# SYSTRAN/faster-whisper

Measured on AMD Instinct MI355X. Metric: audio-sec/sec (RTF) large-v3 fp16 beam=5 batch=16, higher is better.
Workload: dtype f16

## Files before the change

faster_whisper_amd/_lib.py:

```python
import ctypes as C
import os

import numpy as np

_HERE = os.path.dirname(os.path.abspath(__file__))
LIB_PATH = os.environ.get("FWAMD_LIB") or os.path.join(_HERE, "libfwamd.so")

FW_OK = 0
FW_EINVAL = -1
FW_ENODEV = -2
FW_ENOMEM = -3
FW_ERUNTIME = -4
FW_ENOSPC = -5

COMPUTE_FLOAT16 = 0
COMPUTE_INT8_FLOAT16 = 1
FW_DT_F32 = 0
FW_DT_F16 = 1
FW_MAX_ALIGN_HEADS = 64


class FwConfig(C.Structure):
    _fields_ = [
        ("n_mels", C.c_int32), ("n_audio_ctx", C.c_int32), ("d_model", C.c_int32), ("n_heads", C.c_int32),
        ("n_enc_layers", C.c_int32), ("n_dec_layers", C.c_int32), ("n_vocab", C.c_int32),
        ("n_text_ctx", C.c_int32), ("is_multilingual", C.c_int32),
        ("tok_eot", C.c_int32), ("tok_sot", C.c_int32), ("tok_lang_begin", C.c_int32), ("n_langs", C.c_int32),
        ("tok_translate", C.c_int32), ("tok_transcribe", C.c_int32), ("tok_sot_lm", C.c_int32),
        ("tok_sot_prev", C.c_int32), ("tok_no_speech", C.c_int32), ("tok_no_timestamps", C.c_int32),
        ("tok_timestamp_begin", C.c_int32),
        ("n_suppress_begin", C.c_int32), ("suppress_begin", C.c_int32 * 8),
        ("n_align_heads", C.c_int32), ("align_heads", C.c_int32 * (2 * FW_MAX_ALIGN_HEADS)),
    ]


class FwWeight(C.Structure):
    _fields_ = [("name", C.c_char_p), ("data", C.c_void_p), ("dtype", C.c_int32), ("ndim", C.c_int32),
                ("dims", C.c_int64 * 4)]


class FwGenOpts(C.Structure):
    _fields_ = [
        ("beam_size", C.c_int32), ("patience", C.c_float), ("num_hypotheses", C.c_int32),
        ("length_penalty", C.c_float), ("repetition_penalty", C.c_float), ("no_repeat_ngram_size", C.c_int32),
        ("max_length", C.c_int32), ("return_scores", C.c_int32), ("return_no_speech_prob", C.c_int32),
        ("max_initial_timestamp_index", C.c_int32), ("suppress_blank", C.c_int32),
        ("suppress_tokens", C.POINTER(C.c_int32)), ("n_suppress_tokens", C.c_int32),
        ("sampling_topk", C.c_int32), ("sampling_temperature", C.c_float), ("seed", C.c_uint64),
        ("min_new_tokens", C.c_int32),
    ]


class FwVadWeights(C.Structure):
    _fields_ = [
        ("stft_basis", C.c_void_p), ("conv_w", C.c_void_p * 4), ("conv_b", C.c_void_p * 4),
        ("lstm_w", C.c_void_p), ("lstm_r", C.c_void_p), ("lstm_b", C.c_void_p), ("dec_w", C.c_void_p),
        ("dec_b", C.c_float),
    ]


SYMBOLS = [
    "fw_last_error", "fw_abi_version", "fw_device_count",
    "fw_model_create", "fw_model_free", "fw_model_info", "fw_model_blob", "fw_model_create_from_blob_dev",
    "fw_model_set_decode_batch", "fw_model_decode_batch", "fw_model_join_decoder", "fw_model_decode_stats",
    "fw_model_set_merge_wait", "fw_model_set_decode_lanes", "fw_model_run_capacity", "fw_dec_big_min_rows", "fw_dec_big_min_rows_of", "fw_test_knob",
    "fw_test_idle_lead_chunks",
    "fw_pack_blob_size", "fw_pack_blob_copy", "fw_pack_blob_free",
    "fw_logmel", "fw_logmel_full",
    "fw_encode", "fw_encode_pcm", "fw_encode_pcm_dev", "fw_tensor_shape", "fw_tensor_to_host",
    "fw_tensor_from_host", "fw_tensor_free",
    "fw_generate", "fw_detect_language", "fw_align",
    "fw_prof_enable", "fw_prof_reset", "fw_prof_count", "fw_prof_name", "fw_prof_get", "fw_synchronize",
    "fw_dev_alloc", "fw_dev_free", "fw_dev_upload",
    "fw_test_gemm", "fw_test_layernorm", "fw_test_attention", "fw_test_dec_linear", "fw_test_dec_logits", "fw_test_logits_rules",
    "fw_test_dec_self_attn", "fw_test_dec_cross_attn", "fw_test_dec_cross_probs", "fw_test_dec_softmax_pick", "fw_bench_gemm", "fw_bench_dec_linear", "fw_bench_attention",
    "fw_bench_gemm_epi", "fw_bench_dec_linear_epi",
    "fw_vad_create", "fw_vad_forward", "fw_vad_free", "fw_vad_forward_dev", "fw_vad_forward_audio_dev",
    "fw_flac_info", "fw_flac_decode",
    "fw_resample_filter", "fw_resample_dev", "fw_bench_resample",
]

_lib = None


class FwError(RuntimeError):
    pass


def load():
    global _lib
    if _lib is not None:
        return _lib
    if not os.path.exists(LIB_PATH):
        raise FwError(
            f"{LIB_PATH} not found: build it with `python -c 'import __graft_entry__ as g; g.build()'` "
            "(hipcc --offload-arch=gfx950). faster_whisper_amd has no CPU fallback.")
    lib = C.CDLL(LIB_PATH)
    vp, i32, i64, f32p = C.c_void_p, C.c_int32, C.c_int64, C.POINTER(C.c_float)
    i32p, i64p = C.POINTER(C.c_int32), C.POINTER(C.c_int64)
    lib.fw_last_error.restype = C.c_char_p
    lib.fw_abi_version.restype = i32
    lib.fw_device_count.restype = i32
    lib.fw_model_create.argtypes = [C.POINTER(FwConfig), C.POINTER(FwWeight), i32, i32, i32, i32, i32, C.POINTER(vp)]
    lib.fw_model_free.argtypes = [vp]
    lib.fw_model_free.restype = None
    lib.fw_model_info.argtypes = [vp, C.POINTER(FwConfig), i32p, i32p, i32p, i32p]
    lib.fw_model_blob.argtypes = [vp, C.POINTER(vp), i64p]
    lib.fw_model_create_from_blob_dev.argtypes = [C.POINTER(FwConfig), vp, i64, i32, i32, i32, i32, C.POINTER(vp)]
    lib.fw_model_set_decode_batch.argtypes = [vp, i32]
    lib.fw_model_decode_batch.argtypes = [vp]
    lib.fw_model_decode_batch.restype = i32
    lib.fw_model_run_capacity.argtypes = [vp]
    lib.fw_model_run_capacity.restype = i32
    lib.fw_dec_big_min_rows.restype = i32
    if hasattr(lib, "fw_dec_big_min_rows_of"):
        lib.fw_dec_big_min_rows_of.restype = i32
        lib.fw_dec_big_min_rows_of.argtypes = [i32, i32]
    if hasattr(lib, "fw_flac_info"):
        lib.fw_flac_info.argtypes = [vp, i64, i32p, i32p, i32p, i64p]
        lib.fw_flac_decode.argtypes = [vp, i64, vp, i64, i64p, i32p]
    if hasattr(lib, "fw_test_knob"):
        lib.fw_test_knob.argtypes = [i32, i32]
    if hasattr(lib, "fw_test_idle_lead_chunks"):
        lib.fw_test_idle_lead_chunks.argtypes = [i64, i32, i32, i64, i32]
        lib.fw_test_idle_lead_chunks.restype = i64
    lib.fw_model_join_decoder.argtypes = [vp, vp]
    lib.fw_model_set_merge_wait.argtypes = [vp, i32, i32]
    lib.fw_model_set_decode_lanes.argtypes = [vp, i32]
    lib.fw_model_decode_stats.argtypes = [vp, i64p, i64p, i64p, i32p]
    lib.fw_pack_blob_size.argtypes = [C.POINTER(FwConfig), C.POINTER(FwWeight), i32, i32, i64p, C.POINTER(vp)]
    lib.fw_pack_blob_copy.argtypes = [vp, vp, i64]
    lib.fw_pack_blob_free.argtypes = [vp]
    lib.fw_pack_blob_free.restype = None
    lib.fw_logmel.argtypes = [vp, vp, i64p, i32, vp, i32p]
    lib.fw_logmel_full.argtypes = [vp, vp, i64, vp, i64]
    lib.fw_encode.argtypes = [vp, vp, i32, C.POINTER(vp)]
    lib.fw_encode_pcm.argtypes = [vp, vp, i64p, i32, C.POINTER(vp)]
    lib.fw_encode_pcm_dev.argtypes = [vp, vp, i64p, i32, C.POINTER(vp)]
    lib.fw_tensor_shape.argtypes = [vp, i32p, i32p, i32p]
    lib.fw_tensor_to_host.argtypes = [vp, vp, vp]
    lib.fw_tensor_from_host.argtypes = [vp, vp, i32, C.POINTER(vp)]
    lib.fw_tensor_free.argtypes = [vp]
    lib.fw_tensor_free.restype = None
    lib.fw_generate.argtypes = [vp, vp, i32p, i32p, i32, C.POINTER(FwGenOpts), i32p, i32p, f32p, f32p]
    lib.fw_detect_language.argtypes = [vp, vp, i32, i32p, f32p]
    lib.fw_align.argtypes = [vp, vp, i32p, i32, i32p, i32p, i32p, i32, i32, i32, i32p, i32p, f32p]
    lib.fw_prof_enable.argtypes = [vp, i32]
    lib.fw_prof_enable.restype = None
    lib.fw_prof_reset.argtypes = [vp]
    lib.fw_prof_reset.restype = None
    lib.fw_prof_count.restype = i32
    lib.fw_prof_name.argtypes = [i32]
    lib.fw_prof_name.restype = C.c_char_p
    lib.fw_prof_get.argtypes = [vp, i32, C.POINTER(C.c_double), i64p, C.POINTER(C.c_double), C.POINTER(C.c_double)]
    lib.fw_synchronize.argtypes = [vp]
    lib.fw_dev_alloc.argtypes = [vp, i64, C.POINTER(vp)]
    lib.fw_dev_free.argtypes = [vp, vp]
    lib.fw_dev_upload.argtypes = [vp, vp, vp, i64]
    lib.fw_test_gemm.argtypes = [vp, vp, vp, vp, vp, i32, i32, i32, i32, i32, vp]
    lib.fw_test_dec_linear.argtypes = [vp, vp, vp, vp, vp, vp, vp, i32, i32, i32, i32, i32, vp, vp]
    lib.fw_test_dec_logits.argtypes = [vp, vp, i32, vp]
    lib.fw_test_logits_rules.argtypes = [vp, vp, i32, vp, i32, vp, C.POINTER(FwGenOpts), i32, vp, vp]
    if hasattr(lib, "fw_test_dec_self_attn"):
        lib.fw_test_dec_self_attn.argtypes = [vp, vp, vp, vp, vp, i32, i32, i32, i32, i32, i32, i32, i32, i32, i32, i32, vp]
        lib.fw_test_dec_cross_attn.argtypes = [vp, vp, vp, vp, i32, i32, i32, i32, i32, i32, vp, vp, i32, C.c_float, vp]
        lib.fw_test_dec_cross_probs.argtypes = [vp, vp, vp, i32, i32, i32, vp, i32, i32, i32, i32, vp]
        lib.fw_test_dec_softmax_pick.argtypes = [vp, vp, i32, i32, i32, vp, i32, vp]
    lib.fw_bench_attention.argtypes = [vp, i32, i32, i32, i32, i32, f32p]
    lib.fw_bench_gemm.argtypes = [vp, i32, i32, i32, i32, i32, i32, i32, i32, f32p]
    lib.fw_bench_dec_linear.argtypes = [vp, i32, i32, i32, i32, i32, i32, f32p]
    if hasattr(lib, "fw_bench_gemm_epi"):
        lib.fw_bench_gemm_epi.argtypes = [vp, i32, i32, i32, i32, i32, i32, i32, i32, i32, i32, i32, f32p]
        lib.fw_bench_dec_linear_epi.argtypes = [vp, i32, i32, i32, i32, i32, i32, i32, i32, i32, f32p]
    lib.fw_test_layernorm.argtypes = [vp, vp, vp, vp, i32, i32, vp]
    lib.fw_test_attention.argtypes = [vp, vp, vp, vp, i32, i32, i32, vp]
    lib.fw_vad_create.argtypes = [C.POINTER(FwVadWeights), C.POINTER(vp)]
    lib.fw_vad_forward.argtypes = [vp, vp, i64, i32, vp, vp, vp]
    lib.fw_vad_free.argtypes = [vp]
    lib.fw_vad_forward_dev.argtypes = [vp, i32, vp, i64, vp, vp, vp]
    if hasattr(lib, "fw_vad_forward_audio_dev"):
        lib.fw_vad_forward_audio_dev.argtypes = [vp, i32, vp, i64, vp, vp, vp]
    lib.fw_vad_free.restype = None
    if hasattr(lib, "fw_resample_dev"):
        f64 = C.c_double
        lib.fw_resample_filter.argtypes = [i32, i32, i32, f64, vp, i64p, i32p, i32p]
        lib.fw_resample_dev.argtypes = [i32, vp, i64, i32, i32, i32, f64, i32, vp, i64]
        lib.fw_bench_resample.argtypes = [i32, vp, i64, i32, i32, i32, f64, i32, i32, f32p]
    _lib = lib
    return lib


def check(rc: int):
    if rc == FW_OK:
        return
    msg = load().fw_last_error().decode("utf-8", "replace")
    if rc in (FW_EINVAL, FW_ENOSPC):
        raise ValueError(msg)
    raise RuntimeError(f"libfwamd error {rc}: {msg}")


def ptr(a: np.ndarray):
    return a.ctypes.data_as(C.c_void_p)


def as_i32p(a: np.ndarray):
    return a.ctypes.data_as(C.POINTER(C.c_int32))


def as_i64p(a: np.ndarray):
    return a.ctypes.data_as(C.POINTER(C.c_int64))


def as_f32p(a: np.ndarray):
    return a.ctypes.data_as(C.POINTER(C.c_float))
```

faster_whisper_amd/csrc/dec_kernels.hip:

```cpp
#include "common.h"
#include "dec_kernels.h"
#include <stdlib.h>
#include <atomic>
#include <type_traits>

namespace fwd {
static std::atomic<int> g_self_attn_form{0};
static std::atomic<int> g_forms_epoch{0};
static std::atomic<int> g_cross_regs{0};
}

__device__ __forceinline__ size_t frag_off(int row, int k, int KS) {
  return ((size_t)((row >> 4) * KS + (k >> 5)) * 64 + ((k >> 3) & 3) * 16 + (row & 15)) * 8 + (k & 7);
}

__global__ void dec_embed_kernel(const int* __restrict__ tok, const half_t* __restrict__ emb,
                                 const half_t* __restrict__ pos_emb, half_t* __restrict__ x,
                                 half_t* __restrict__ xfrag, int d, const int* __restrict__ d_step, int pos_fixed,
                                 int P, int blk_n) {
  const int r = blockIdx.x;
  const int pos = blk_n > 0 ? pos_fixed + r % blk_n : (pos_fixed >= 0 ? pos_fixed : P - 1 + *d_step);
  const half2_t* e = reinterpret_cast<const half2_t*>(emb + (size_t)tok[r] * d);
  const half2_t* pe = reinterpret_cast<const half2_t*>(pos_emb + (size_t)pos * d);
  half2_t* xo = reinterpret_cast<half2_t*>(x + (size_t)r * d);
// ... 818 lines not shown
      src[j] = c * Kbeam + kvidx[pc];
      kv[j] = *reinterpret_cast<const half8_t*>(kbase + src[j] * slot_stride + (size_t)pc * 64);
    }
#pragma unroll
    for (int j = 0; j < 4; ++j) {
      const int p = p0 + 8 * j + pg;
      const float sc = dot8(kv[j]);
      if (p < pos) {
        if (cc == 0) { sp[p] = sc; ssrc[p] = src[j]; }
        mx = fmaxf(mx, sc);
      }
    }
  }
  mx = wave_max(mx);
  __builtin_amdgcn_wave_barrier();
  float sum = 0.f;
  for (int p = lane; p < pos; p += 64) {
    const float e = __expf(sp[p] - mx);
    sp[p] = e;
    sum += e;
  }
  const float e_new = __expf(s_new - mx);
  sum = wave_sum(sum) + e_new;
  __builtin_amdgcn_wave_barrier();
  float acc[8];
#pragma unroll
  for (int e = 0; e < 8; ++e) acc[e] = 0.f;
  const half_t* vb = vc + h * head_stride + cc * 8;
#pragma unroll 4
  for (int p = pg; p < pos; p += 8) {
    const half8_t vv = *reinterpret_cast<const half8_t*>(vb + ssrc[p] * slot_stride + (size_t)p * 64);
    const float w = sp[p];
#pragma unroll
    for (int e = 0; e < 8; ++e) acc[e] += w * (float)vv[e];
  }
#pragma unroll
  for (int e = 0; e < 8; ++e) {
    float a = acc[e];
    a += __shfl_xor(a, 8, 64);
    a += __shfl_xor(a, 16, 64);
    a += __shfl_xor(a, 32, 64);
    acc[e] = a;
  }
  if (pg == 0) {
    const float inv = 1.f / sum;
    half8_t o;
#pragma unroll
    for (int e = 0; e < 8; ++e) o[e] = (half_t)((acc[e] + e_new * (float)vn8[e]) * inv);
    half_t* dst = frag ? out + frag_off(r, h * 64 + cc * 8, d >> 5) : out + (size_t)r * d + h * 64 + cc * 8;
    *reinterpret_cast<half8_t*>(dst) = o;
  }
}

template <int U, bool PIPE, int MAXT, bool PB = false>
__global__ __launch_bounds__(MAXT) void dec_self_attn2_kernel(const half_t* __restrict__ qkv, int d, half_t* __restrict__ kc,
                                                             half_t* __restrict__ vc, int n_ctx, int cache_ctx,
                                                             int H, const uint8_t* __restrict__ kvidx2, int Kbeam, int kmul,
                                                             half_t* __restrict__ out, const int* __restrict__ d_step,
                                                             int pos_fixed, int P, int R_total, int frag) {
  extern __shared__ float sa_smem[];
  constexpr int NB = 4 * U;
  const int lane = threadIdx.x & 63;
  const int wave = __builtin_amdgcn_readfirstlane(threadIdx.x >> 6);
  float* sp = sa_smem + (size_t)wave * 2 * n_ctx;
  int* ssrc = reinterpret_cast<int*>(sp + n_ctx);
  const int h = blockIdx.x, c = blockIdx.y;
  const int r = c * kmul + wave, kb = PB ? 0 : wave;
  const int step = PB ? 0 : *d_step;
  const int pos = PB ? pos_fixed + wave : (pos_fixed >= 0 ? pos_fixed : P - 1 + step);
  const int slot = c * Kbeam + kb;
  const int cur = (pos_fixed >= 0) ? 0 : (step & 1);
  const uint8_t* kvidx = kvidx2 + ((size_t)cur * R_total + slot) * n_ctx;
  const half_t* qr = qkv + (size_t)r * 3 * d + h * 64;
  const size_t head_stride = (size_t)cache_ctx * 64;
  const size_t slot_stride = (size_t)H * head_stride;
  const int pg = lane >> 3, cc = lane & 7;
  for (int p4 = 4 * lane; p4 < pos; p4 += 256) {
    const unsigned w = PB ? 0u : *reinterpret_cast<const unsigned*>(kvidx + p4);
    intx4 s4;
    s4[0] = c * Kbeam + (int)(w & 0xffu); s4[1] = c * Kbeam + (int)((w >> 8) & 0xffu);
    s4[2] = c * Kbeam + (int)((w >> 16) & 0xffu); s4[3] = c * Kbeam + (int)(w >> 24);
    *reinterpret_cast<intx4*>(ssrc + p4) = s4;
  }
  const half8_t q8 = *reinterpret_cast<const half8_t*>(qr + cc * 8);
  const half8_t kn8 = *reinterpret_cast<const half8_t*>(qr + d + cc * 8);
  const half8_t vn8 = *reinterpret_cast<const half8_t*>(qr + 2 * d + cc * 8);
  float q[8];
#pragma unroll
  for (int e = 0; e < 8; ++e) q[e] = (float)q8[e] * 0.125f;
  if (pg == 0) {
    *reinterpret_cast<half8_t*>(kc + slot * slot_stride + h * head_stride + (size_t)pos * 64 + cc * 8) = kn8;
    *reinterpret_cast<half8_t*>(vc + slot * slot_stride + h * head_stride + (size_t)pos * 64 + cc * 8) = vn8;
  }
  auto dot8 = [&](const half8_t& k) {
    float sacc = 0.f;
#pragma unroll
    for (int e = 0; e < 8; ++e) sacc = __builtin_fmaf(q[e], (float)k[e], sacc);
    return sum8_dpp(sacc);
  };
  const float s_new = dot8(kn8);
  float mx = s_new;
  __builtin_amdgcn_wave_barrier();
  const char* kbase = reinterpret_cast<const char*>(kc + h * head_stride);
  const char* vbase = reinterpret_cast<const char*>(vc + h * head_stride);
  const unsigned slot_bytes = (unsigned)(slot_stride * sizeof(half_t));
  struct Batch { half8_t row[NB]; };
  auto fetch = [&](Batch& b, const char* base, int p0, const half_t* sib) {
#pragma unroll
    for (int j = 0; j < NB; ++j) {
      const int p = p0 + 8 * j + pg;
      const int pc = p < pos ? p : pos - 1;
      const unsigned off = (unsigned)ssrc[pc] * slot_bytes + (unsigned)(pc * 128 + cc * 16);
      if (PB && pc >= pos_fixed)
        b.row[j] = *reinterpret_cast<const half8_t*>(sib + (size_t)(pc - pos_fixed) * 3 * d + cc * 8);
      else
        b.row[j] = *reinterpret_cast<const half8_t*>(base + off);
    }
  };
  const half_t* ksib = qkv + (size_t)c * kmul * 3 * d + d + h * 64;
  const half_t* vsib = ksib + d;
  auto score = [&](const Batch& b, int p0) {
#pragma unroll
    for (int j = 0; j < NB; ++j) {
      const int p = p0 + 8 * j + pg;
      const float sc = dot8(b.row[j]);
      if (p < pos) {
        if (cc == 0) sp[p] = sc;
        mx = fmaxf(mx, sc);
      }
    }
  };
  Batch b0, b1;
  if (pos > 0) {
    fetch(b0, kbase, 0, ksib);
    for (int p0 = 0; p0 < pos; p0 += 16 * NB) {
      if (PIPE) {
        fetch(b1, kbase, p0 + 8 * NB, ksib);
        score(b0, p0);
        fetch(b0, kbase, p0 + 16 * NB, ksib);
        score(b1, p0 + 8 * NB);
      } else {
        score(b0, p0);
        if (p0 + 8 * NB < pos) {
          fetch(b0, kbase, p0 + 8 * NB, ksib);
          score(b0, p0 + 8 * NB);
          if (p0 + 16 * NB < pos) fetch(b0, kbase, p0 + 16 * NB, ksib);
        }
      }
    }
    fetch(b0, vbase, 0, vsib);
  }
  mx = wave_max_v(mx);
  __builtin_amdgcn_wave_barrier();
  float sum = 0.f;
  for (int p = lane; p < pos; p += 64) {
    const float e = __expf(sp[p] - mx);
    sp[p] = e;
    sum += e;
  }
  const float e_new = __expf(s_new - mx);
  sum = wave_sum_v(sum) + e_new;
  __builtin_amdgcn_wave_barrier();
  float acc[8];
#pragma unroll
  for (int e = 0; e < 8; ++e) acc[e] = 0.f;
  auto accum = [&](const Batch& b, int p0) {
#pragma unroll
    for (int j = 0; j < NB; ++j) {
      const int p = p0 + 8 * j + pg;
      if (p < pos) {
        const float w = sp[p];
#pragma unroll
        for (int e = 0; e < 8; ++e) acc[e] = __builtin_fmaf(w, (float)b.row[j][e], acc[e]);
      }
    }
  };
  for (int p0 = 0; p0 < pos; p0 += 16 * NB) {
    if (PIPE) {
      fetch(b1, vbase, p0 + 8 * NB, vsib);
      accum(b0, p0);
      fetch(b0, vbase, p0 + 16 * NB, vsib);
      accum(b1, p0 + 8 * NB);
    } else {
      accum(b0, p0);
      if (p0 + 8 * NB < pos) {
        fetch(b0, vbase, p0 + 8 * NB, vsib);
        accum(b0, p0 + 8 * NB);
        if (p0 + 16 * NB < pos) fetch(b0, vbase, p0 + 16 * NB, vsib);
      }
    }
  }
#pragma unroll
  for (int e = 0; e < 8; ++e) acc[e] = sum_x8_x16_x32_v(acc[e]);
  if (pg == 0) {
    const float inv = 1.f / sum;
    half8_t o;
#pragma unroll
    for (int e = 0; e < 8; ++e) o[e] = (half_t)((acc[e] + e_new * (float)vn8[e]) * inv);
    half_t* dst = frag ? out + frag_off(r, h * 64 + cc * 8, d >> 5) : out + (size_t)r * d + h * 64 + cc * 8;
    *reinterpret_cast<half8_t*>(dst) = o;
  }
}

template <int CA_WAVES, bool NTL, int MINW = 1>
__global__ __launch_bounds__(CA_WAVES * 64, MINW) void dec_cross_attn_kernel(const half_t* __restrict__ qx, int d,
                                                             const half_t* __restrict__ ck,
                                                             const half_t* __restrict__ cvt, int T, int kvp,
                                                             int kmul, half_t* __restrict__ out,
                                                             const int* __restrict__ done, int kv_div, int frag,
                                                             const int* __restrict__ slot_map) {
  __shared__ float sm[CA_WAVES][16], sl[CA_WAVES][16];
  __shared__ float so[CA_WAVES][16][65];
  const int h = blockIdx.x, c = blockIdx.y;
  if (done && done[c]) return;
  const int tid = threadIdx.x, lane = tid & 63, wave = tid >> 6;
  const int j = lane & 15, g = lane >> 4;
  const int ce = slot_map[c / kv_div];
  const half_t* kbase = ck + ((size_t)ce * (d >> 6) + h) * kvp * 64 + lane * 8;
  const half_t* vbase = cvt + ((size_t)ce * (d >> 6) + h) * kvp * 64 + lane * 8;
  half8_t qf[2];
  {
    if (j < kmul) {
      const half_t* qp = qx + (size_t)(c * kmul + j) * d + h * 64 + g * 8;
#pragma unroll
      for (int s = 0; s < 2; ++s) {
        half8_t v = *reinterpret_cast<const half8_t*>(qp + s * 32);
#pragma unroll
        for (int e = 0; e < 8; ++e) v[e] = v[e] * (half_t)0.125f;
        qf[s] = v;
      }
    } else {
      qf[0] = half8_t{0, 0, 0, 0, 0, 0, 0, 0};
      qf[1] = qf[0];
    }
  }
  floatx4 o[4];
#pragma unroll
  for (int dt = 0; dt < 4; ++dt) o[dt] = floatx4{0, 0, 0, 0};
  float m_run = -1.0e30f, l_run = 0.f;
  const float LOG2E = 1.4426950408889634f;
  const int ngroups = (T + 31) >> 5;
  auto load_kv = [&](int gi, half8_t (&kf)[4], half8_t (&vf)[4]) {
    const half_t* kp = kbase + (size_t)gi * 2048;
    const half_t* vp = vbase + (size_t)gi * 2048;
#pragma unroll
    for (int q = 0; q < 4; ++q)
      kf[q] = NTL ? __builtin_nontemporal_load(reinterpret_cast<const half8_t*>(kp + q * 512))
                  : *reinterpret_cast<const half8_t*>(kp + q * 512);
#pragma unroll
    for (int dt = 0; dt < 4; ++dt)
      vf[dt] = NTL ? __builtin_nontemporal_load(reinterpret_cast<const half8_t*>(vp + dt * 512))
// ... 670 lines not shown
    if (K >= 2560)
      dec_gemm_frag_i8_kernel<8, 4, 4, 3><<<g4, 512, 0, st>>>(xq, x_scale, Wq, w_scale, bias, res, ldr, out, ldo, R, N, K, act);
    else
      dec_gemm_frag_i8_kernel<4, 4, 4, 5><<<g4, 256, 0, st>>>(xq, x_scale, Wq, w_scale, bias, res, ldr, out, ldo, R, N, K, act);
    return 0;
  }
  const dim3 grid(N / 32, ((R + 15) / 16 + 1) / 2);
  if (K >= 2560)
    dec_gemm_frag_i8_kernel<8, 2, 2><<<grid, 512, 0, st>>>(xq, x_scale, Wq, w_scale, bias, res, ldr, out, ldo, R, N, K, act);
  else
    dec_gemm_frag_i8_kernel<4, 2, 2><<<grid, 256, 0, st>>>(xq, x_scale, Wq, w_scale, bias, res, ldr, out, ldo, R, N, K, act);
  return 0;
}

template <bool I8, bool LNF, int RT>
static void wave_go(hipStream_t st, const void* xf, const float* x_scale, const void* Wf, const float* w_scale,
                    const float* s1, const float* cf, float* out, int ldo, int R, int N, int K) {
  constexpr int NT = 2, WM = 1, WN = 4;
  const int n_rt = (R + 15) / 16, n_ct = (N + 15) / 16;
  const int n_cg = ((n_ct + NT * WN - 1) / (NT * WN) + 7) & ~7;
  const int n_rg = (n_rt + RT * WM - 1) / (RT * WM);
  dec_gemm_wave_kernel<I8, LNF, true, RT, NT, WM, WN><<<n_cg * n_rg, WM * WN * 64, 0, st>>>(
      xf, x_scale, Wf, w_scale, nullptr, s1, cf, out, ldo, R, N, K, n_rg);
}

int launch_dec_logits(hipStream_t st, bool i8, const void* xf, const float* x_scale, const void* Wf,
                      const float* w_scale, const float* s1, const float* cf, float* out, int ldo, int R, int N, int K) {
  if (K % (i8 ? 64 : 32) != 0 || R < 1) return -1;
  if (i8 ? (!x_scale || !w_scale) : ((s1 == nullptr) != (cf == nullptr))) return -1;
  const int n_rt = (R + 15) / 16;
#define WG(RT)                                                                                   \
  do {                                                                                           \
    if (i8) wave_go<true, false, RT>(st, xf, x_scale, Wf, w_scale, s1, cf, out, ldo, R, N, K);   \
    else if (s1) wave_go<false, true, RT>(st, xf, x_scale, Wf, w_scale, s1, cf, out, ldo, R, N, K); \
    else wave_go<false, false, RT>(st, xf, x_scale, Wf, w_scale, s1, cf, out, ldo, R, N, K);     \
  } while (0)
  if (n_rt == 1) WG(1);
  else if (n_rt == 2) WG(2);
  else if (n_rt == 3) WG(3);
  else if (n_rt == 4) WG(4);
  else WG(5);
#undef WG
  return 0;
}

bool self_attn_block_ok(int n_ctx, int cache_ctx, int d, int R_total) {
  return (n_ctx & 3) == 0 && (size_t)R_total * cache_ctx * d * sizeof(half_t) < ((size_t)1 << 32);
}

void launch_self_attn(hipStream_t st, const half_t* qkv, int d, half_t* kc, half_t* vc, int n_ctx, int cache_ctx, int H,
                      const uint8_t* kvidx2, int Kbeam, int kmul, half_t* out, int rows, const int* d_step,
                      int pos_fixed, int P, int R_total, int frag, int blk_n) {
  if (blk_n > 0) {
    dec_self_attn2_kernel<1, true, 1024, true><<<dim3(H, rows / blk_n), blk_n * 64, (size_t)blk_n * 2 * n_ctx * sizeof(float), st>>>(
        qkv, d, kc, vc, n_ctx, cache_ctx, H, kvidx2, Kbeam, blk_n, out, d_step, pos_fixed, P, R_total, frag);
    return;
  }
  const dim3 grid(H, rows / kmul);
  const size_t lds = (size_t)kmul * 2 * n_ctx * sizeof(float);
  int form = g_self_attn_form.load(std::memory_order_relaxed);
  if ((n_ctx & 3) != 0 || (size_t)R_total * cache_ctx * d * sizeof(half_t) >= ((size_t)1 << 32)) form = 1;
  if (form == 0) form = (kmul <= 8 && (int)(grid.x * grid.y) <= 768) ? 2 : 3;
  if (form == 2 && kmul > 8) form = 3;
#define SA_ARGS qkv, d, kc, vc, n_ctx, cache_ctx, H, kvidx2, Kbeam, kmul, out, d_step, pos_fixed, P, R_total, frag
  if (form == 1) dec_self_attn_kernel<<<grid, kmul * 64, lds, st>>>(SA_ARGS);
  else if (form == 2) dec_self_attn2_kernel<4, false, 512><<<grid, kmul * 64, lds, st>>>(SA_ARGS);
  else dec_self_attn2_kernel<1, true, 1024><<<grid, kmul * 64, lds, st>>>(SA_ARGS);
#undef SA_ARGS
}
void set_self_attn_form(int form) { g_self_attn_form.store(form); g_forms_epoch.fetch_add(1); }
int kernel_forms_epoch() { return g_forms_epoch.load(); }
void bump_kernel_forms_epoch() { g_forms_epoch.fetch_add(1); }

void launch_cross_attn(hipStream_t st, const half_t* qx, int d, const half_t* ck, const half_t* cvt, int T, int kvp,
                       int kmul, half_t* out, int B, int H, const int* done, int kv_div, int frag, const int* slot_map) {
  const int cap = g_cross_regs.load(std::memory_order_relaxed);
  if (cap == 1)
    dec_cross_attn_kernel<8, true, 5><<<dim3(H, B), 512, 0, st>>>(qx, d, ck, cvt, T, kvp, kmul, out, done, kv_div, frag, slot_map);
  else if (cap == 2)
    dec_cross_attn_kernel<8, true, 6><<<dim3(H, B), 512, 0, st>>>(qx, d, ck, cvt, T, kvp, kmul, out, done, kv_div, frag, slot_map);
  else
    dec_cross_attn_kernel<8, true><<<dim3(H, B), 512, 0, st>>>(qx, d, ck, cvt, T, kvp, kmul, out, done, kv_div, frag, slot_map);
}
void set_cross_attn_regs(int cap) { g_cross_regs.store(cap); g_forms_epoch.fetch_add(1); }

void launch_nospeech(hipStream_t st, const float* logits, int V, int row_mul, int no_speech_id, float* out, int B) {
  dec_nospeech_kernel<<<B, 1024, 0, st>>>(logits, V, row_mul, no_speech_id, out);
}

void launch_logits_process(hipStream_t st, const GenDev& gp, float* logits, const unsigned long long* sup_bits,
                           const int* hist2, const float* cum2, const int* d_step, const int* done, float* cand_val,
                           int* cand_tok) {
  const bool wide = gp.ts_begin >= 48 * LP_THREADS;
#define LP_GO(SMP, TXI) \
  dec_logits_process_kernel<SMP, TXI><<<gp.R, LP_THREADS, 0, st>>>(gp, logits, sup_bits, hist2, cum2, d_step, done, cand_val, cand_tok)
  if (gp.sample) { if (wide) LP_GO(true, 48); else LP_GO(true, 0); }
  else { if (wide) LP_GO(false, 48); else LP_GO(false, 0); }
#undef LP_GO
}

void launch_beam_update(hipStream_t st, const GenDev& gp, const float* cand_val, const int* cand_tok, int* hist2,
                        float* cum2, uint8_t* kvidx2, int* cur_tok, const int* d_step, int* done, int* n_done,
                        int* n_fin, int* fin_tok, int* fin_len, float* fin_score, float* fin_cum) {
  dec_beam_update_kernel<<<gp.B, 64, 0, st>>>(gp, cand_val, cand_tok, hist2, cum2, kvidx2, cur_tok, d_step, done,
                                              n_done, n_fin, fin_tok, fin_len, fin_score, fin_cum);
}

void launch_step_advance(hipStream_t st, int* d_step) { dec_step_advance_kernel<<<1, 1, 0, st>>>(d_step); }

void launch_token_prob(hipStream_t st, const float* logits, int V, const int* target, float* out, int out_stride,
                       int out_off, int rows, int row_mul) {
  dec_token_prob_kernel<<<rows, 1024, 0, st>>>(logits, V, target, out, out_stride, out_off, row_mul);
// ... 11 lines not shown
```

faster_whisper_amd/csrc/engine.hip:

```cpp
#include "engine.h"

#include <math.h>
#include <stdarg.h>
#include <stdio.h>
#include <stdlib.h>
#include <string.h>

#include <algorithm>

#include "dec_kernels.h"
#include "kernels.h"

namespace fw {

static thread_local char g_err[1024] = "";
void set_error(const char* fmt, ...) {
  va_list ap;
  va_start(ap, fmt);
  vsnprintf(g_err, sizeof(g_err), fmt, ap);
  va_end(ap);
}

int dev_alloc(void** p, size_t bytes) {
  if (bytes == 0) bytes = 256;
// ... 2163 lines not shown
  int rc;
  auto cleanup = [&]() { for (half_t* p : {dqk, dvt, dout}) if (p) (void)hipFree(p); };
  if ((rc = dev_alloc_t(&dqk, nqk)) || (rc = dev_alloc_t(&dvt, nvt)) || (rc = dev_alloc_t(&dout, no))) { cleanup(); return rc; }
  {
    std::vector<uint16_t> h(std::max(nqk, nvt));
    uint32_t sd = 777u;
    for (auto& v : h) { sd = sd * 1664525u + 1013904223u; v = f32_to_f16_bits(((int)(sd >> 16) % 2001 - 1000) * 2e-3f); }
    FW_HIP(hipMemcpy(dqk, h.data(), nqk * 2, hipMemcpyHostToDevice));
    FW_HIP(hipMemcpy(dvt, h.data(), nvt * 2, hipMemcpyHostToDevice));
  }
  hipEvent_t e0, e1;
  FW_HIP(hipEventCreate(&e0));
  FW_HIP(hipEventCreate(&e1));
  auto go = [&]() {
    fwk::launch_attn_enc(m->stream, dqk, dqk + d, 2 * d, (int64_t)T * 2 * d, dvt, tp, (int64_t)d * tp, dout, d, (int64_t)T * d, B,
                         H, T, variant);
  };
  go();
  FW_HIP(hipEventRecord(e0, m->stream));
  for (int i = 0; i < iters; ++i) go();
  FW_HIP(hipEventRecord(e1, m->stream));
  hipError_t he = hipEventSynchronize(e1);
  float ms = 0.f;
  if (he == hipSuccess) he = hipEventElapsedTime(&ms, e0, e1);
  (void)hipEventDestroy(e0);
  (void)hipEventDestroy(e1);
  cleanup();
  if (he != hipSuccess) { set_error("attention bench failed: %s", hipGetErrorString(he)); return FW_ERUNTIME; }
  *ms_out = ms / (float)iters;
  return FW_OK;
}

extern "C++" {
namespace {
struct DevBufs {
  std::vector<void*> p;
  template <typename T>
  int alloc(T** dst, size_t n) {
    int rc = dev_alloc_t(dst, n);
    if (!rc) p.push_back(*dst);
    return rc;
  }
  ~DevBufs() { for (void* q : p) (void)hipFree(q); }
};
int upload_f16_to(const float* src, size_t n, half_t* dst) {
  std::vector<uint16_t> tmp(n);
  for (size_t i = 0; i < n; ++i) tmp[i] = f32_to_f16_bits(src[i]);
  FW_HIP(hipMemcpy(dst, tmp.data(), n * 2, hipMemcpyHostToDevice));
  return FW_OK;
}
}
}

int32_t fw_test_dec_self_attn(fw_model* fm, const float* qkv, float* kcache, float* vcache, const uint8_t* kvidx,
                              int32_t n_chunks, int32_t kmul, int32_t Kbeam, int32_t H, int32_t n_ctx, int32_t cache_ctx,
                              int32_t pos_fixed, int32_t P, int32_t step, int32_t blk_n, int32_t frag, float* out) {
  FW_CHECK_ARG(fm && qkv && kcache && vcache && kvidx && out, "null argument");
  FW_CHECK_ARG(n_chunks >= 1 && H >= 1 && kmul >= 1 && kmul <= 16 && Kbeam >= 1 && Kbeam <= 255, "bad geometry");
  FW_CHECK_ARG(n_ctx >= 1 && n_ctx <= 448 && cache_ctx >= 1 && cache_ctx <= n_ctx, "need 1 <= cache_ctx <= n_ctx <= 448");
  FW_CHECK_ARG(blk_n >= 0 && (blk_n == 0 ? kmul <= Kbeam : (kmul == blk_n && pos_fixed >= 0)),
               "blk_n = 0: kmul <= Kbeam; blk_n > 0: kmul == blk_n and pos_fixed >= 0");
  const int pos0 = pos_fixed >= 0 ? pos_fixed : P - 1 + step;
  const int pos_last = pos0 + (blk_n > 0 ? blk_n - 1 : 0);
  FW_CHECK_ARG(pos0 >= 0 && pos_last < cache_ctx, "positions %d..%d outside the cache (%d)", pos0, pos_last, cache_ctx);
  const int d = H * 64, R = n_chunks * kmul, R16 = (R + 15) / 16 * 16, R_total = n_chunks * Kbeam;
  FW_CHECK_ARG(blk_n == 0 || fwd::self_attn_block_ok(n_ctx, cache_ctx, d, R_total), "position blocks need n_ctx %% 4 == 0");
  const size_t n_tab = (size_t)2 * R_total * n_ctx, n_cache = (size_t)R_total * H * cache_ctx * 64;
  for (size_t i = 0; i < n_tab; ++i)
    FW_CHECK_ARG(kvidx[i] < Kbeam, "kvidx[%zu] = %d is not a beam of %d", i, (int)kvidx[i], Kbeam);
  Model* m = &fm->impl;
  std::lock_guard<std::mutex> lk(m->mu);
  FW_HIP(hipSetDevice(m->device));
  DevBufs db;
  half_t *d_qkv, *d_kc, *d_vc, *d_out;
  uint8_t* d_idx;
  int* d_step;
  int rc;
  if ((rc = db.alloc(&d_qkv, (size_t)R * 3 * d)) || (rc = db.alloc(&d_kc, n_cache)) || (rc = db.alloc(&d_vc, n_cache)) ||
      (rc = db.alloc(&d_out, (size_t)R16 * d)) || (rc = db.alloc(&d_idx, n_tab)) || (rc = db.alloc(&d_step, 1)))
    return rc;
  if ((rc = upload_f16_to(qkv, (size_t)R * 3 * d, d_qkv)) || (rc = upload_f16_to(kcache, n_cache, d_kc)) ||
      (rc = upload_f16_to(vcache, n_cache, d_vc)))
    return rc;
  FW_HIP(hipMemcpy(d_idx, kvidx, n_tab, hipMemcpyHostToDevice));
  FW_HIP(hipMemcpy(d_step, &step, sizeof(int), hipMemcpyHostToDevice));
  FW_HIP(hipMemset(d_out, 0, (size_t)R16 * d * 2));
  fwd::launch_self_attn(m->stream, d_qkv, d, d_kc, d_vc, n_ctx, cache_ctx, H, d_idx, Kbeam, kmul, d_out, R, d_step,
                        pos_fixed, P, R_total, frag ? 1 : 0, blk_n);
  FW_HIP(hipGetLastError());
  if ((rc = download_f16(m, d_kc, n_cache, kcache)) || (rc = download_f16(m, d_vc, n_cache, vcache))) return rc;
  if (!frag) return download_f16(m, d_out, (size_t)R * d, out);
  std::vector<float> of((size_t)R16 * d);
  if ((rc = download_f16(m, d_out, of.size(), of.data()))) return rc;
  for (int r = 0; r < R; ++r)
    for (int n = 0; n < d; ++n) out[(size_t)r * d + n] = of[frag_pos(r, n, d, 32)];
  return FW_OK;
}

int32_t fw_test_dec_cross_attn(fw_model* fm, const float* q, const float* k, const float* v, int32_t n_enc, int32_t T,
                               int32_t H, int32_t B, int32_t kmul, int32_t kv_div, const int32_t* slot_map,
                               const int32_t* done, int32_t frag, float k_pad, float* out) {
  FW_CHECK_ARG(fm && q && k && v && slot_map && out, "null argument");
  FW_CHECK_ARG(n_enc >= 1 && T >= 1 && H >= 1 && B >= 1 && kmul >= 1 && kmul <= 16 && kv_div >= 1, "bad geometry");
  const int n_map = (B + kv_div - 1) / kv_div;
  for (int i = 0; i < n_map; ++i)
    FW_CHECK_ARG(slot_map[i] >= 0 && slot_map[i] < n_enc, "slot_map[%d] = %d outside [0, %d)", i, slot_map[i], n_enc);
// ... 99 lines not shown
```

Measured before the change: 3193.

## Precompute byte offsets in LDS table and trim decoder self-attention inner loop

```diff
diff --git a/faster_whisper_amd/_lib.py b/faster_whisper_amd/_lib.py
--- a/faster_whisper_amd/_lib.py
+++ b/faster_whisper_amd/_lib.py
@@ -74,7 +74,7 @@
     "fw_dev_alloc", "fw_dev_free", "fw_dev_upload",
     "fw_test_gemm", "fw_test_layernorm", "fw_test_attention", "fw_test_dec_linear", "fw_test_dec_logits", "fw_test_logits_rules",
     "fw_test_dec_self_attn", "fw_test_dec_cross_attn", "fw_test_dec_cross_probs", "fw_test_dec_softmax_pick", "fw_bench_gemm", "fw_bench_dec_linear", "fw_bench_attention",
-    "fw_bench_gemm_epi", "fw_bench_dec_linear_epi",
+    "fw_bench_gemm_epi", "fw_bench_dec_linear_epi", "fw_bench_dec_self_attn",
     "fw_vad_create", "fw_vad_forward", "fw_vad_free", "fw_vad_forward_dev", "fw_vad_forward_audio_dev",
     "fw_flac_info", "fw_flac_decode",
     "fw_resample_filter", "fw_resample_dev", "fw_bench_resample",
@@ -172,6 +172,8 @@
     if hasattr(lib, "fw_bench_gemm_epi"):
         lib.fw_bench_gemm_epi.argtypes = [vp, i32, i32, i32, i32, i32, i32, i32, i32, i32, i32, i32, f32p]
         lib.fw_bench_dec_linear_epi.argtypes = [vp, i32, i32, i32, i32, i32, i32, i32, i32, i32, f32p]
+    if hasattr(lib, "fw_bench_dec_self_attn"):
+        lib.fw_bench_dec_self_attn.argtypes = [vp, i32, i32, i32, i32, i32, i32, i32, f32p]
     lib.fw_test_layernorm.argtypes = [vp, vp, vp, vp, i32, i32, vp]
     lib.fw_test_attention.argtypes = [vp, vp, vp, vp, i32, i32, i32, vp]
     lib.fw_vad_create.argtypes = [C.POINTER(FwVadWeights), C.POINTER(vp)]
diff --git a/faster_whisper_amd/csrc/dec_kernels.hip b/faster_whisper_amd/csrc/dec_kernels.hip
--- a/faster_whisper_amd/csrc/dec_kernels.hip
+++ b/faster_whisper_amd/csrc/dec_kernels.hip
@@ -894,8 +894,10 @@
   }
 }
 
+static __host__ __device__ __forceinline__ int sa2_table_len(int n_ctx) { return ((n_ctx + 127) & ~127) + 32; }
+static __host__ __device__ __forceinline__ int sa2_lds_words(int n_ctx) { return ((n_ctx + 7) & ~7) + sa2_table_len(n_ctx); }
 template <int U, bool PIPE, int MAXT, bool PB = false>
-__global__ __launch_bounds__(MAXT) void dec_self_attn2_kernel(const half_t* __restrict__ qkv, int d, half_t* __restrict__ kc,
+__global__ __launch_bounds__(MAXT, (U == 1 && !PB) ? 8 : 1) void dec_self_attn2_kernel(const half_t* __restrict__ qkv, int d, half_t* __restrict__ kc,
                                                              half_t* __restrict__ vc, int n_ctx, int cache_ctx,
                                                              int H, const uint8_t* __restrict__ kvidx2, int Kbeam, int kmul,
                                                              half_t* __restrict__ out, const int* __restrict__ d_step,
@@ -904,8 +906,8 @@
   constexpr int NB = 4 * U;
   const int lane = threadIdx.x & 63;
   const int wave = __builtin_amdgcn_readfirstlane(threadIdx.x >> 6);
-  float* sp = sa_smem + (size_t)wave * 2 * n_ctx;
-  int* ssrc = reinterpret_cast<int*>(sp + n_ctx);
+  float* sp = sa_smem + (size_t)wave * sa2_lds_words(n_ctx);
+  int* ssrc = reinterpret_cast<int*>(sp + ((n_ctx + 7) & ~7));
   const int h = blockIdx.x, c = blockIdx.y;
   const int r = c * kmul + wave, kb = PB ? 0 : wave;
   const int step = PB ? 0 : *d_step;
@@ -916,13 +918,27 @@
   const half_t* qr = qkv + (size_t)r * 3 * d + h * 64;
   const size_t head_stride = (size_t)cache_ctx * 64;
   const size_t slot_stride = (size_t)H * head_stride;
+  const unsigned slot_bytes = (unsigned)(slot_stride * sizeof(half_t));
   const int pg = lane >> 3, cc = lane & 7;
-  for (int p4 = 4 * lane; p4 < pos; p4 += 256) {
-    const unsigned w = PB ? 0u : *reinterpret_cast<const unsigned*>(kvidx + p4);
-    intx4 s4;
-    s4[0] = c * Kbeam + (int)(w & 0xffu); s4[1] = c * Kbeam + (int)((w >> 8) & 0xffu);
-    s4[2] = c * Kbeam + (int)((w >> 16) & 0xffu); s4[3] = c * Kbeam + (int)(w >> 24);
-    *reinterpret_cast<intx4*>(ssrc + p4) = s4;
+  if constexpr (PB) {
+    for (int p4 = 4 * lane; p4 < pos; p4 += 256) {
+      intx4 s4;
+#pragma unroll
+      for (int i = 0; i < 4; ++i) s4[i] = (int)((unsigned)(c * Kbeam) * slot_bytes + (unsigned)(p4 + i) * 128u);
+      *reinterpret_cast<intx4*>(ssrc + p4) = s4;
+    }
+  } else if (pos > 0) {
+    const int ext = PIPE ? ((pos + 16 * NB - 1) & ~(16 * NB - 1)) + 8 * NB : (pos + 8 * NB - 1) & ~(8 * NB - 1);
+    const unsigned last = (unsigned)(c * Kbeam + kvidx[pos - 1]) * slot_bytes + (unsigned)(pos - 1) * 128u;
+    for (int p4 = 4 * lane; p4 < ext; p4 += 256) {
+      const unsigned w = p4 < pos ? *reinterpret_cast<const unsigned*>(kvidx + p4) : 0u;
+      intx4 s4;
+#pragma unroll
+      for (int i = 0; i < 4; ++i)
+        s4[i] = p4 + i < pos ? (int)((unsigned)(c * Kbeam + (int)((w >> (8 * i)) & 0xffu)) * slot_bytes + (unsigned)(p4 + i) * 128u)
+                             : (int)last;
+      *reinterpret_cast<intx4*>(ssrc + p4) = s4;
+    }
   }
   const half8_t q8 = *reinterpret_cast<const half8_t*>(qr + cc * 8);
   const half8_t kn8 = *reinterpret_cast<const half8_t*>(qr + d + cc * 8);
@@ -943,33 +959,47 @@
   const float s_new = dot8(kn8);
   float mx = s_new;
   __builtin_amdgcn_wave_barrier();
-  const char* kbase = reinterpret_cast<const char*>(kc + h * head_stride);
-  const char* vbase = reinterpret_cast<const char*>(vc + h * head_stride);
-  const unsigned slot_bytes = (unsigned)(slot_stride * sizeof(half_t));
+  const unsigned head_bytes = (unsigned)h * ((unsigned)cache_ctx * 128u);
+  const char* kbase = reinterpret_cast<const char*>(kc) + head_bytes;
+  const char* vbase = reinterpret_cast<const char*>(vc) + head_bytes;
   struct Batch { half8_t row[NB]; };
   auto fetch = [&](Batch& b, const char* base, int p0, const half_t* sib) {
 #pragma unroll
     for (int j = 0; j < NB; ++j) {
       const int p = p0 + 8 * j + pg;
-      const int pc = p < pos ? p : pos - 1;
-      const unsigned off = (unsigned)ssrc[pc] * slot_bytes + (unsigned)(pc * 128 + cc * 16);
-      if (PB && pc >= pos_fixed)
-        b.row[j] = *reinterpret_cast<const half8_t*>(sib + (size_t)(pc - pos_fixed) * 3 * d + cc * 8);
-      else
-        b.row[j] = *reinterpret_cast<const half8_t*>(base + off);
+      if constexpr (PB) {
+        const int pc = p < pos ? p : pos - 1;
+        if (pc >= pos_fixed)
+          b.row[j] = *reinterpret_cast<const half8_t*>(sib + (size_t)(pc - pos_fixed) * 3 * d + cc * 8);
+        else
+          b.row[j] = *reinterpret_cast<const half8_t*>(base + ((unsigned)ssrc[pc] + (unsigned)(cc * 16)));
+      } else {
+        b.row[j] = *reinterpret_cast<const half8_t*>(base + ((unsigned)ssrc[p] + (unsigned)(cc * 16)));
+      }
     }
   };
   const half_t* ksib = qkv + (size_t)c * kmul * 3 * d + d + h * 64;
   const half_t* vsib = ksib + d;
-  auto score = [&](const Batch& b, int p0) {
-#pragma unroll
-    for (int j = 0; j < NB; ++j) {
-      const int p = p0 + 8 * j + pg;
-      const float sc = dot8(b.row[j]);
+  auto score_row = [&](const half8_t& k, int p) {
+    const float sc = dot8(k);
+    if constexpr (PB) {
       if (p < pos) {
         if (cc == 0) sp[p] = sc;
         mx = fmaxf(mx, sc);
       }
+    } else {
+      sp[p] = sc;
+      mx = fmaxf(mx, sc);
+    }
+  };
+  auto score = [&](const Batch& b, int p0) {
+    if (PB || p0 + 8 * NB <= pos) {
+#pragma unroll
+      for (int j = 0; j < NB; ++j) score_row(b.row[j], p0 + 8 * j + pg);
+    } else {
+#pragma unroll
+      for (int j = 0; j < NB; ++j)
+        if (p0 + 8 * j < pos) score_row(b.row[j], p0 + 8 * j + pg);
     }
   };
   Batch b0, b1;
@@ -978,13 +1008,16 @@
     for (int p0 = 0; p0 < pos; p0 += 16 * NB) {
       if (PIPE) {
         fetch(b1, kbase, p0 + 8 * NB, ksib);
+        __builtin_amdgcn_sched_barrier(0);
         score(b0, p0);
         fetch(b0, kbase, p0 + 16 * NB, ksib);
+        __builtin_amdgcn_sched_barrier(0);
         score(b1, p0 + 8 * NB);
       } else {
         score(b0, p0);
         if (p0 + 8 * NB < pos) {
           fetch(b0, kbase, p0 + 8 * NB, ksib);
+          __builtin_amdgcn_sched_barrier(0);
           score(b0, p0 + 8 * NB);
           if (p0 + 16 * NB < pos) fetch(b0, kbase, p0 + 16 * NB, ksib);
         }
@@ -1000,33 +1033,51 @@
     sp[p] = e;
     sum += e;
   }
+  if (!PB && lane < 8 && (pos & ~7) + lane >= pos) sp[(pos & ~7) + lane] = 0.f;
   const float e_new = __expf(s_new - mx);
   sum = wave_sum_v(sum) + e_new;
   __builtin_amdgcn_wave_barrier();
   float acc[8];
 #pragma unroll
   for (int e = 0; e < 8; ++e) acc[e] = 0.f;
+  auto accum_row = [&](const half8_t& v, int p) {
+    if (PB && p >= pos) return;
+    const float w = sp[p];
+    if constexpr (PB) {
+#pragma unroll
+      for (int e = 0; e < 8; ++e) acc[e] = __builtin_fmaf(w, (float)v[e], acc[e]);
+    } else {
+      const intx4 u = __builtin_bit_cast(intx4, v);
+#pragma unroll
+      for (int e = 0; e < 4; ++e) {
+        asm("v_fma_mix_f32 %0, %1, %2, %0 op_sel_hi:[0,1,0]" : "+v"(acc[2 * e]) : "v"(w), "v"(u[e]));
+        asm("v_fma_mix_f32 %0, %1, %2, %0 op_sel:[0,1,0] op_sel_hi:[0,1,0]" : "+v"(acc[2 * e + 1]) : "v"(w), "v"(u[e]));
+      }
+    }
+  };
   auto accum = [&](const Batch& b, int p0) {
-#pragma unroll
-    for (int j = 0; j < NB; ++j) {
-      const int p = p0 + 8 * j + pg;
-      if (p < pos) {
-        const float w = sp[p];
-#pragma unroll
-        for (int e = 0; e < 8; ++e) acc[e] = __builtin_fmaf(w, (float)b.row[j][e], acc[e]);
-      }
+    if (PB || p0 + 8 * NB <= pos) {
+#pragma unroll
+      for (int j = 0; j < NB; ++j) accum_row(b.row[j], p0 + 8 * j + pg);
+    } else {
+#pragma unroll
+      for (int j = 0; j < NB; ++j)
+        if (p0 + 8 * j < pos) accum_row(b.row[j], p0 + 8 * j + pg);
     }
   };
   for (int p0 = 0; p0 < pos; p0 += 16 * NB) {
     if (PIPE) {
       fetch(b1, vbase, p0 + 8 * NB, vsib);
+      __builtin_amdgcn_sched_barrier(0);
       accum(b0, p0);
       fetch(b0, vbase, p0 + 16 * NB, vsib);
+      __builtin_amdgcn_sched_barrier(0);
       accum(b1, p0 + 8 * NB);
     } else {
       accum(b0, p0);
       if (p0 + 8 * NB < pos) {
         fetch(b0, vbase, p0 + 8 * NB, vsib);
+        __builtin_amdgcn_sched_barrier(0);
         accum(b0, p0 + 8 * NB);
         if (p0 + 16 * NB < pos) fetch(b0, vbase, p0 + 16 * NB, vsib);
       }
@@ -1035,10 +1086,13 @@
 #pragma unroll
   for (int e = 0; e < 8; ++e) acc[e] = sum_x8_x16_x32_v(acc[e]);
   if (pg == 0) {
+    unsigned voff = (unsigned)(2 * d + cc * 8);
+    asm volatile("" : "+v"(voff));
+    const half8_t vn = *reinterpret_cast<const half8_t*>(qr + voff);
     const float inv = 1.f / sum;
     half8_t o;
 #pragma unroll
-    for (int e = 0; e < 8; ++e) o[e] = (half_t)((acc[e] + e_new * (float)vn8[e]) * inv);
+    for (int e = 0; e < 8; ++e) o[e] = (half_t)((acc[e] + e_new * (float)vn[e]) * inv);
     half_t* dst = frag ? out + frag_off(r, h * 64 + cc * 8, d >> 5) : out + (size_t)r * d + h * 64 + cc * 8;
     *reinterpret_cast<half8_t*>(dst) = o;
   }
@@ -1815,12 +1869,12 @@
                       const uint8_t* kvidx2, int Kbeam, int kmul, half_t* out, int rows, const int* d_step,
                       int pos_fixed, int P, int R_total, int frag, int blk_n) {
   if (blk_n > 0) {
-    dec_self_attn2_kernel<1, true, 1024, true><<<dim3(H, rows / blk_n), blk_n * 64, (size_t)blk_n * 2 * n_ctx * sizeof(float), st>>>(
+    dec_self_attn2_kernel<1, true, 1024, true><<<dim3(H, rows / blk_n), blk_n * 64, (size_t)blk_n * sa2_lds_words(n_ctx) * sizeof(float), st>>>(
         qkv, d, kc, vc, n_ctx, cache_ctx, H, kvidx2, Kbeam, blk_n, out, d_step, pos_fixed, P, R_total, frag);
     return;
   }
   const dim3 grid(H, rows / kmul);
-  const size_t lds = (size_t)kmul * 2 * n_ctx * sizeof(float);
+  const size_t lds = (size_t)kmul * sa2_lds_words(n_ctx) * sizeof(float);
   int form = g_self_attn_form.load(std::memory_order_relaxed);
   if ((n_ctx & 3) != 0 || (size_t)R_total * cache_ctx * d * sizeof(half_t) >= ((size_t)1 << 32)) form = 1;
   if (form == 0) form = (kmul <= 8 && (int)(grid.x * grid.y) <= 768) ? 2 : 3;
diff --git a/faster_whisper_amd/csrc/engine.hip b/faster_whisper_amd/csrc/engine.hip
--- a/faster_whisper_amd/csrc/engine.hip
+++ b/faster_whisper_amd/csrc/engine.hip
@@ -2239,6 +2239,68 @@
 }
 }
 
+int32_t fw_bench_dec_self_attn(fw_model* fm, int32_t n_chunks, int32_t kmul, int32_t H, int32_t cache_ctx, int32_t pos_lo,
+                               int32_t pos_hi, int32_t reps, float* us_out) {
+  FW_CHECK_ARG(fm && us_out && n_chunks >= 1 && kmul >= 1 && kmul <= 16 && H >= 1 && reps >= 1, "bad argument");
+  FW_CHECK_ARG(pos_lo >= 0 && pos_lo <= pos_hi && pos_hi < cache_ctx && cache_ctx <= 448, "need 0 <= pos_lo <= pos_hi < cache_ctx <= 448");
+  const int n_ctx = 448, d = H * 64, R = n_chunks * kmul, R16 = (R + 15) / 16 * 16;
+  const size_t n_cache = (size_t)R * H * cache_ctx * 64;
+  FW_CHECK_ARG(n_cache * 2 < ((size_t)1 << 32), "a cache of %zu bytes needs the first form: not what this measures", n_cache * 2);
+  const int n_sets = (int)std::max<size_t>(2, (((size_t)640 << 20) + 4 * n_cache - 1) / (4 * n_cache));
+  Model* m = &fm->impl;
+  std::lock_guard<std::mutex> lk(m->mu);
+  FW_HIP(hipSetDevice(m->device));
+  DevBufs db;
+  half_t *d_qkv, *d_kc, *d_vc, *d_out;
+  uint8_t* d_idx;
+  int* d_step;
+  int rc;
+  if ((rc = db.alloc(&d_qkv, (size_t)R * 3 * d)) || (rc = db.alloc(&d_kc, n_cache * n_sets)) || (rc = db.alloc(&d_vc, n_cache * n_sets)) ||
+      (rc = db.alloc(&d_out, (size_t)R16 * d)) || (rc = db.alloc(&d_idx, (size_t)2 * R * n_ctx)) || (rc = db.alloc(&d_step, 1)))
+    return rc;
+  {
+    std::vector<uint16_t> h(std::max(n_cache, (size_t)R * 3 * d));
+    uint32_t sd = 2463534242u;
+    for (auto& v : h) { sd = sd * 1664525u + 1013904223u; v = f32_to_f16_bits(((int)(sd >> 16) % 2001 - 1000) * 1e-3f); }
+    for (int c = 0; c < n_sets; ++c) {
+      FW_HIP(hipMemcpy(d_kc + (size_t)c * n_cache, h.data(), n_cache * 2, hipMemcpyHostToDevice));
+      FW_HIP(hipMemcpy(d_vc + (size_t)c * n_cache, h.data(), n_cache * 2, hipMemcpyHostToDevice));
+    }
+    FW_HIP(hipMemcpy(d_qkv, h.data(), (size_t)R * 3 * d * 2, hipMemcpyHostToDevice));
+    std::vector<uint8_t> idx((size_t)2 * R * n_ctx);
+    for (size_t i = 0; i < idx.size(); ++i) {
+      const int p = (int)(i % n_ctx), beam = (int)((i / n_ctx) % kmul);
+      idx[i] = (uint8_t)((p & 15) < 14 ? 0 : beam);
+    }
+    FW_HIP(hipMemcpy(d_idx, idx.data(), idx.size(), hipMemcpyHostToDevice));
+  }
+  FW_HIP(hipMemset(d_step, 0, sizeof(int)));
+  hipEvent_t e0, e1;
+  FW_HIP(hipEventCreate(&e0));
+  FW_HIP(hipEventCreate(&e1));
+  hipStream_t st = m->stream;
+  int n = 0;
+  auto sweep = [&]() {
+    for (int pos = pos_lo; pos <= pos_hi; ++pos, ++n)
+      fwd::launch_self_attn(st, d_qkv, d, d_kc + (size_t)(n % n_sets) * n_cache, d_vc + (size_t)(n % n_sets) * n_cache, n_ctx,
+                            cache_ctx, H, d_idx, kmul, kmul, d_out, R, d_step, pos, 0, R, 1, 0);
+  };
+  sweep();
+  n = 0;
+  FW_HIP(hipEventRecord(e0, st));
+  for (int i = 0; i < reps; ++i) sweep();
+  FW_HIP(hipEventRecord(e1, st));
+  hipError_t he = hipEventSynchronize(e1);
+  if (he == hipSuccess) he = hipGetLastError();
+  float ms = 0.f;
+  if (he == hipSuccess) he = hipEventElapsedTime(&ms, e0, e1);
+  (void)hipEventDestroy(e0);
+  (void)hipEventDestroy(e1);
+  if (he != hipSuccess) { set_error("fw_bench_dec_self_attn: %s", hipGetErrorString(he)); return FW_ENODEV; }
+  *us_out = ms * 1000.f / (float)n;
+  return FW_OK;
+}
+
 int32_t fw_test_dec_self_attn(fw_model* fm, const float* qkv, float* kcache, float* vcache, const uint8_t* kvidx,
                               int32_t n_chunks, int32_t kmul, int32_t Kbeam, int32_t H, int32_t n_ctx, int32_t cache_ctx,
                               int32_t pos_fixed, int32_t P, int32_t step, int32_t blk_n, int32_t frag, float* out) {
diff --git a/profiles/dec_self_attn_bench.py b/profiles/dec_self_attn_bench.py
--- /dev/null
+++ b/profiles/dec_self_attn_bench.py
@@ -0,0 +1,38 @@
+import argparse
+import ctypes as C
+import os
+import sys
+
+sys.path.insert(0, os.path.dirname(os.path.dirname(os.path.abspath(__file__))))
+from faster_whisper_amd import Whisper, _lib, get_config, synthetic_weights
+
+GEOMS = [("merged 160 x 5", 160), ("solo 16 x 5", 16)]
+
+
+def main():
+    ap = argparse.ArgumentParser()
+    ap.add_argument("--form", type=int, default=0)
+    ap.add_argument("--reps", type=int, default=10, help="sweeps over the positions per measurement")
+    ap.add_argument("--n", type=int, default=3, help="measurements per geometry")
+    a = ap.parse_args()
+    cfg = get_config("micro")
+    m = Whisper("synthetic:micro", device="cuda", files={"config": cfg, "weights": synthetic_weights(cfg, seed=1)},
+                max_batch_size=1, max_beam_size=1)
+    h = m._replicas[0].handle
+    us = C.c_float()
+    _lib.check(m._lib.fw_test_knob(2, a.form))
+    try:
+        print(f"lib {os.environ.get('FWAMD_LIB', 'in-tree')}  form {a.form}  positions 4 .. 103, H 20, cache_ctx 104")
+        for name, n_chunks in GEOMS:
+            t = []
+            for _ in range(a.n):
+                _lib.check(m._lib.fw_bench_dec_self_attn(h, n_chunks, 5, 20, 104, 4, 103, a.reps, C.byref(us)))
+                t.append(us.value)
+            print("  %-16s us per launch %s   min %.2f  max %.2f  spread %.2f" %
+                  (name, " ".join("%7.2f" % x for x in t), min(t), max(t), max(t) - min(t)), flush=True)
+    finally:
+        _lib.check(m._lib.fw_test_knob(2, 0))
+
+
+if __name__ == "__main__":
+    main()
```

Result: no change. 3198 (median of 2 runs) (+0.2%).
